# zkHubHQ/distributed-groth16

Hardware: AMD Instinct MI355X
Metric: groth16_constraints_per_sec (higher is better)
Workload: dtype u32; 1 GPU; BN254 Groth16 prove from the matrices, synthetic R1CS with 2^20 - 2 constraints (3 nonzeros per row of A and B), 2^20 wires, 2 instance variables; r, s != 0 (R1CS x witness + 6 NTTs of 2^20 + 4 G1 MSMs + 1 G2 MSM); proving key RESIDENT as window tables (built once per key outside the timed region); curve=bn254, log_domain=20, parallelism=single GPU, key_table_bytes=6039807360, key_table_stride=1

## Files before the change

### distributed-groth16_amd/csrc/ntt.hip

```cpp
#include <cstdio>
#include <cstdlib>
#include "ctx.h"
#include "fp29.h"
#include "types.h"

namespace dg16 {

static void optional_table_skipped(const char* what, size_t bytes) {
  static const bool verbose = [] { const char* e = getenv("DG16_VERBOSE"); return e && atoi(e) != 0; }();
  if (verbose) fprintf(stderr, "[dg16] %s (%zu bytes) not built: hipMalloc failed; using the composed form\n", what, bytes);
}


constexpr unsigned kTileLog = 10;
constexpr unsigned kTile = 1u << kTileLog;
constexpr unsigned kMaxStepLog = 10;
constexpr unsigned kLoBits = 11;

template <class F>
struct StepArgs {
  const F* src[3];
  F* dst[3];
  unsigned log_n, s, log_a, log_b;
  unsigned last;
  unsigned log_n1, log_n2;
  const F* small;
  unsigned sm;
  const F* tw_lo;
  const F* tw_hi;
  unsigned lb;
  const F* tw_full;
  const F* post_full;
  const F* pre_lo;
  const F* pre_hi;
  const F* post_lo;
  const F* post_hi;
  unsigned plb;
  const F* scale;
  unsigned src_piece_log, dst_piece_log;
  size_t src_piece_stride, dst_piece_stride;
};

__device__ __forceinline__ unsigned bitrev(unsigned v, unsigned bits) {
  return bits ? (__brev(v) >> (32 - bits)) : 0;
}

constexpr int kNttBound = 48 * 64;
constexpr int kNttIn = 128;
constexpr int kNttFirstOut = 9 * 64;
constexpr int kNttStepGrowth = 6 * 64 + 32;
constexpr int kNttOddGrowth = 3 * 64 + 32;
static_assert(kNttFirstOut + (int)((kMaxStepLog - 2) / 2) * kNttStepGrowth + kNttOddGrowth <= kNttBound,
              "NTT tile bound: a pass of kMaxStepLog levels can exceed kNttBound");

template <class F>
__global__ void __launch_bounds__(256) ntt_step_kernel(StepArgs<F> p) {
  using P = typename F::Params;
  using T = RR<P>;
  constexpr int N = T::N;
  using El = Fe<P, kNttBound, 1>;
  using Tw = Fe<P, 64, 1>;
  __shared__ uint32_t tile_w[kTile * N];
  constexpr int NLW = T::NL;
  __shared__ uint32_t tw_w[(1u << (kMaxStepLog - 1)) * NLW];
  static_assert((1u << (kMaxStepLog - 2)) * N <= (1u << (kMaxStepLog - 1)) * NLW, "unpacked twiddles of the shorter steps fit");
  const unsigned tid = threadIdx.x;
  const unsigned s = p.s;
  const unsigned nj = 1u << s;
  const unsigned log_t = (p.log_n < kTileLog ? p.log_n : kTileLog) - s;
  const unsigned Tn = 1u << log_t;
  const unsigned elems = nj << log_t;
  const size_t tile_id = blockIdx.x;
  auto slot = [](unsigned e) { return (e ^ ((e >> 2) & 31u)) * (unsigned)N; };
  auto ld_tile = [&](unsigned i) {
    El v;
    const unsigned o = slot(i);
#pragma unroll
    for (int j = 0; j < N; j++) v.l[j] = tile_w[o + j];
    return v;
  };
  auto st_tile = [&](unsigned i, const El& v) {
    const unsigned o = slot(i);
#pragma unroll
    for (int j = 0; j < N; j++) tile_w[o + j] = v.l[j];
  };
  const bool tw_packed = p.s == kMaxStepLog;
  auto ld_tw = [&](unsigned i) {
    if (tw_packed) return fe_from_words<P>(&tw_w[i * NLW]);
    Tw v;
#pragma unroll
    for (int j = 0; j < N; j++) v.l[j] = tw_w[i * N + j];
    return v;
  };
  auto ld_packed = [&](const F* ptr) { return fe_from_words<P>(ptr->l); };

  size_t a = 0, b0 = 0, k1_0 = 0, k2 = 0;
  if (!p.last) {
    const unsigned tiles_per_a_log = p.log_b - log_t;
    a = tile_id >> tiles_per_a_log;
    b0 = (tile_id & (((size_t)1 << tiles_per_a_log) - 1)) << log_t;
  } else {
    const unsigned k1_tiles_log = p.log_n1 - log_t;
    k2 = tile_id >> k1_tiles_log;
    k1_0 = (tile_id & (((size_t)1 << k1_tiles_log) - 1)) << log_t;
  }

  if (s >= 1)
    for (unsigned t = tid; t < (nj >> 1); t += 256) {
      const F* w = p.small + ((size_t)t << (p.sm - s));
      if (tw_packed) {
#pragma unroll
        for (int j = 0; j < NLW; j++) tw_w[t * NLW + j] = w->l[j];
      } else {
        const Tw u = ld_packed(w);
#pragma unroll
        for (int j = 0; j < N; j++) tw_w[t * N + j] = u.l[j];
      }
    }

  for (unsigned idx = tid; idx < elems; idx += 256) {
    unsigned n, t;
    size_t g;
    if (!p.last) {
      t = idx & (Tn - 1);
      n = idx >> log_t;
      g = ((((a << s) + n) << p.log_b) + b0 + t);
    } else {
      n = idx & (nj - 1);
      t = idx >> s;
      g = ((((k1_0 + t) << p.log_n2) + k2) << s) + n;
    }
    const size_t gs = p.src_piece_stride ? (g >> p.src_piece_log) * p.src_piece_stride + (g & (((size_t)1 << p.src_piece_log) - 1)) : g;
    const Tw x = ld_packed(p.src[blockIdx.y] + gs);
    El v = x.template as<kNttBound, 1>();
    if (p.pre_lo) {
      const auto w = ld_packed(p.pre_lo + (g & ((1u << p.plb) - 1))) * ld_packed(p.pre_hi + (g >> p.plb));
      v = (x * w).template as<kNttBound, 1>();
    }
    st_tile((bitrev(n, s) << log_t) + t, v);
  }
  __syncthreads();

  unsigned lv = 1;
  if (s >= 2) {
    using In = Fe<P, kNttIn, 1>;
    const Tw w3 = ld_tw(1u << (s - 2));
    for (unsigned q = tid; q < (elems >> 2); q += 256) {
      const unsigned t = q & (Tn - 1), pi = q >> log_t;
      const unsigned ia = (pi << (2 + log_t)) + t;
      const In xa = ld_tile(ia).template unsafe_assume<kNttIn, 1>(), xb = ld_tile(ia + Tn).template unsafe_assume<kNttIn, 1>(),
               xc = ld_tile(ia + 2 * Tn).template unsafe_assume<kNttIn, 1>(), xd = ld_tile(ia + 3 * Tn).template unsafe_assume<kNttIn, 1>();
      const auto a1 = xa + xb;
      const auto b1 = xa - xb;
      const auto c1 = xc + xd;
      const auto te = (xc - xd) * w3;
      const auto o0 = a1 + c1;
      const auto o2 = a1 - c1;
      const auto o1 = b1 + te;
      const auto o3 = b1 - te;
      static_assert(decltype(o0)::Bound <= kNttFirstOut && decltype(o1)::Bound <= kNttFirstOut &&
                    decltype(o2)::Bound <= kNttFirstOut && decltype(o3)::Bound <= kNttFirstOut, "first radix-4 step bound");
      st_tile(ia, norm(o0).template as<kNttBound, 1>());
      st_tile(ia + 2 * Tn, norm(o2).template as<kNttBound, 1>());
      st_tile(ia + Tn, norm(o1).template as<kNttBound, 1>());
      st_tile(ia + 3 * Tn, norm(o3).template as<kNttBound, 1>());
    }
    __syncthreads();
    lv = 3;
  }
  for (; lv + 1 <= s; lv += 2) {
    const unsigned half = 1u << (lv - 1);
    const unsigned sh1 = s - lv, sh2 = s - lv - 1;
    for (unsigned q = tid; q < (elems >> 2); q += 256) {
      const unsigned t = q & (Tn - 1), pi = q >> log_t;
      const unsigned k = pi & (half - 1), blk = pi >> (lv - 1);
      const unsigned ia = ((((blk << (lv + 1)) + k)) << log_t) + t;
      const unsigned st = half << log_t;
      const El xa = ld_tile(ia), xb = ld_tile(ia + st), xc = ld_tile(ia + 2 * st), xd = ld_tile(ia + 3 * st);
      const Tw w1 = ld_tw(k << sh1);
      const auto tb = xb * w1;
      const auto td = xd * w1;
      const auto a1 = xa + tb;
      const auto b1 = xa - tb;
      const auto c1 = xc + td;
      const auto d1 = xc - td;
      const auto tc = c1 * ld_tw(k << sh2);
      const auto te = d1 * ld_tw((k + half) << sh2);
      const auto o0 = a1 + tc;
      const auto o2 = a1 - tc;
      const auto o1 = b1 + te;
      const auto o3 = b1 - te;
      static_assert(decltype(o0)::Bound - kNttBound <= kNttStepGrowth && decltype(o1)::Bound - kNttBound <= kNttStepGrowth &&
                    decltype(o2)::Bound - kNttBound <= kNttStepGrowth && decltype(o3)::Bound - kNttBound <= kNttStepGrowth,
                    "radix-4 step growth");
      st_tile(ia, norm(o0).template unsafe_assume<kNttBound, 1>());
      st_tile(ia + 2 * st, norm(o2).template unsafe_assume<kNttBound, 1>());
      st_tile(ia + st, norm(o1).template unsafe_assume<kNttBound, 1>());
      st_tile(ia + 3 * st, norm(o3).template unsafe_assume<kNttBound, 1>());
    }
    __syncthreads();
  }
  if (lv == s) {
    const unsigned half = 1u << (s - 1);
    for (unsigned q = tid; q < (elems >> 1); q += 256) {
      const unsigned t = q & (Tn - 1), k = q >> log_t;
      const unsigned i0 = (k << log_t) + t, i1 = i0 + (half << log_t);
      const El x = ld_tile(i0);
      const auto ty = ld_tile(i1) * ld_tw(k);
      const auto o0 = x + ty;
      const auto o1 = x - ty;
      static_assert(decltype(o0)::Bound - kNttBound <= kNttOddGrowth && decltype(o1)::Bound - kNttBound <= kNttOddGrowth,
                    "odd level growth");
      st_tile(i0, norm(o0).template unsafe_assume<kNttBound, 1>());
      st_tile(i1, norm(o1).template unsafe_assume<kNttBound, 1>());
    }
    __syncthreads();
  }

  for (unsigned idx = tid; idx < elems; idx += 256) {
    unsigned t = idx & (Tn - 1);
    unsigned k = idx >> log_t;
    const El v = ld_tile((k << log_t) + t);
    Fe<P, 64, 1> out;
    size_t g;
    if (!p.last) {
      size_t b = b0 + t;
      size_t e = (b * k) << p.log_a;
      if (p.tw_full) {
        if (e || p.scale) out = canon(v * ld_packed(p.tw_full + (((size_t)k << p.log_b) + b)));
        else out = canon(v);
      } else if (e) {
        const auto w = ld_packed(p.tw_lo + (e & ((1u << p.lb) - 1))) * ld_packed(p.tw_hi + (e >> p.lb));
        out = canon(v * w);
      } else if (p.scale) {
        out = canon(v * ld_packed(p.tw_hi));
      } else {
        out = canon(v);
      }
      g = ((((a << s) + k) << p.log_b) + b);
    } else {
      g = (k1_0 + t) + (k2 << p.log_n1) + ((size_t)k << (p.log_n1 + p.log_n2));
      if (p.post_full) {
        const auto w = ld_packed(p.post_full + g);
        if (p.scale) out = canon((v * ld_packed(p.scale)) * w);
        else out = canon(v * w);
      } else if (p.scale && p.post_lo) {
        const auto w = ld_packed(p.post_lo + (g & ((1u << p.plb) - 1))) * ld_packed(p.post_hi + (g >> p.plb));
        out = canon((v * ld_packed(p.scale)) * w);
      } else if (p.scale) {
        out = canon(v * ld_packed(p.scale));
      } else if (p.post_lo) {
        const auto w = ld_packed(p.post_lo + (g & ((1u << p.plb) - 1))) * ld_packed(p.post_hi + (g >> p.plb));
        out = canon(v * w);
      } else {
        out = canon(v);
      }
    }
    F o;
    fe_to_words<P>(out, o.l);
    if (p.dst_piece_stride) g = (g >> p.dst_piece_log) * p.dst_piece_stride + (g & (((size_t)1 << p.dst_piece_log) - 1));
    p.dst[blockIdx.y][g] = o;
  }
}

template <class F>
__global__ void to_internal_kernel(F* t, size_t count) {
  size_t j = (size_t)blockIdx.x * blockDim.x + threadIdx.x;
  if (j >= count) return;
  using P = typename F::Params;
  F c;
#pragma unroll
  for (int i = 0; i < F::NL; i++) c.l[i] = RR<P>::R_WORDS.v[i];
  t[j] = t[j] * c;
}
template <class F>
static void* internal_copy(hipStream_t s, const void* src, size_t count) {
  void* d = nullptr;
  DG_HIP(hipMalloc(&d, count * sizeof(F)));
  DG_HIP(hipMemcpyAsync(d, src, count * sizeof(F), hipMemcpyDeviceToDevice, s));
  hipLaunchKernelGGL(to_internal_kernel<F>, dim3((unsigned)((count + 255) / 256)), dim3(256), 0, s, (F*)d, count);
  return d;
}

template <class F>
__global__ void powers_kernel(F* out, size_t count, unsigned shift, const F* base_ptr,
                              unsigned root_log, int invert, const F* c_ptr) {
  size_t j = (size_t)blockIdx.x * blockDim.x + threadIdx.x;
  if (j >= count) return;
  F base;
  if (base_ptr) {
    base = *base_ptr;
  } else {
    F w;
#pragma unroll
    for (int i = 0; i < F::NL; i++) w.l[i] = F::Params::TWO_ADIC_ROOT[i];
    for (unsigned i = root_log; i < (unsigned)F::Params::TWO_ADICITY; i++) w = w.sqr();
    if (invert) {
      F acc = F::one(), sq = w;
      for (unsigned i = 0; i < root_log; i++) { acc = acc * sq; sq = sq.sqr(); }
      w = acc;
    }
    base = w;
  }
  F r = base.pow_u64((uint64_t)j << shift);
  if (c_ptr) r = r * *c_ptr;
  out[j] = r;
}

template <class F>
__global__ void n_inv_kernel(F* out, unsigned log_n) {
  F two = F::one() + F::one();
  F half = two.inv();
  *out = half.pow_u64(log_n);
}

struct Plan {
  unsigned nsteps;
  unsigned s[3];
};
static Plan make_plan(unsigned log_n) {
  Plan pl{};
  if (log_n <= kTileLog && log_n <= kMaxStepLog) {
    pl.nsteps = 1;
    pl.s[0] = log_n;
  } else if (log_n <= 2 * kMaxStepLog) {
    pl.nsteps = 2;
    pl.s[0] = log_n / 2;
    pl.s[1] = log_n - pl.s[0];
  } else {
    pl.nsteps = 3;
    pl.s[0] = log_n / 3;
    pl.s[1] = (log_n - pl.s[0]) / 2;
    pl.s[2] = log_n - pl.s[0] - pl.s[1];
  }
  return pl;
}

constexpr unsigned kFullTwiddleMaxLog = 24;
inline unsigned full_twiddle_min_log() {
  static const unsigned v = [] { const char* e = getenv("DG16_NTT_TABLE_MIN_LOG"); return e ? (unsigned)atoi(e) : 21u; }();
  return v;
}
template <class F>
__global__ void __launch_bounds__(256) full_twiddle_kernel(F* __restrict__ out, size_t count, unsigned log_a, unsigned log_b,
                                                            const F* __restrict__ lo, const F* __restrict__ hi, unsigned lb) {
  using P = typename F::Params;
  const size_t idx = (size_t)blockIdx.x * blockDim.x + threadIdx.x;
  if (idx >= count) return;
  const size_t k = idx >> log_b, b = idx & (((size_t)1 << log_b) - 1);
  const size_t e = (b * k) << log_a;
  const auto w = fe_from_words<P>(lo[e & (((size_t)1 << lb) - 1)].l) * fe_from_words<P>(hi[e >> lb].l);
  F o;
  fe_to_words<P>(canon(w), o.l);
  out[idx] = o;
}
template <class F>
__global__ void __launch_bounds__(256) flat_powers_kernel(F* __restrict__ out, size_t count, const F* __restrict__ lo,
                                                           const F* __restrict__ hi, unsigned lb) {
  using P = typename F::Params;
  const size_t o = (size_t)blockIdx.x * blockDim.x + threadIdx.x;
  if (o >= count) return;
  const auto w = fe_from_words<P>(lo[o & (((size_t)1 << lb) - 1)].l) * fe_from_words<P>(hi[o >> lb].l);
  F r;
  fe_to_words<P>(canon(w), r.l);
  out[o] = r;
}

template <class F>
static const TwiddleSet& get_twiddles(Call& k, int curve, unsigned log_n, int inverse) {
  std::lock_guard<std::mutex> g(k.ctx->mu);
  TwiddleKey key{curve, log_n, inverse};
  auto it = k.ctx->twiddles.find(key);
  if (it != k.ctx->twiddles.end()) return it->second;
  TwiddleSet ts;
  ts.lb = log_n < kLoBits ? log_n : kLoBits;
  ts.sm = log_n < kMaxStepLog ? (log_n ? log_n : 1) : kMaxStepLog;
  size_t nlo = (size_t)1 << ts.lb, nhi = (size_t)1 << (log_n - ts.lb), nsm = (size_t)1 << (ts.sm - 1);
  DG_HIP(hipMalloc(&ts.lo, nlo * sizeof(F)));
  DG_HIP(hipMalloc(&ts.hi, nhi * sizeof(F)));
  DG_HIP(hipMalloc(&ts.small, nsm * sizeof(F)));
  DG_HIP(hipMalloc(&ts.n_inv, sizeof(F)));
  hipStream_t s = k.s();
  hipLaunchKernelGGL(n_inv_kernel<F>, dim3(1), dim3(1), 0, s, (F*)ts.n_inv, log_n);
  hipLaunchKernelGGL(powers_kernel<F>, dim3((unsigned)((nlo + 255) / 256)), dim3(256), 0, s, (F*)ts.lo,
                     nlo, 0u, (const F*)nullptr, log_n, inverse, (const F*)nullptr);
  hipLaunchKernelGGL(powers_kernel<F>, dim3((unsigned)((nhi + 255) / 256)), dim3(256), 0, s, (F*)ts.hi,
                     nhi, ts.lb, (const F*)nullptr, log_n, inverse, (const F*)nullptr);
  if (inverse) {
    DG_HIP(hipMalloc(&ts.hi_scaled, nhi * sizeof(F)));
    hipLaunchKernelGGL(powers_kernel<F>, dim3((unsigned)((nhi + 255) / 256)), dim3(256), 0, s,
                       (F*)ts.hi_scaled, nhi, ts.lb, (const F*)nullptr, log_n, inverse,
                       (const F*)ts.n_inv);
  }
  hipLaunchKernelGGL(powers_kernel<F>, dim3((unsigned)((nsm + 255) / 256)), dim3(256), 0, s, (F*)ts.small,
                     nsm, log_n >= ts.sm ? log_n - ts.sm : 0, (const F*)nullptr, log_n ? log_n : 1, inverse,
                     (const F*)nullptr);
  ts.lo_i = internal_copy<F>(s, ts.lo, nlo);
  ts.hi_i = internal_copy<F>(s, ts.hi, nhi);
  if (inverse) ts.hi_scaled_i = internal_copy<F>(s, ts.hi_scaled, nhi);
  ts.small_i = internal_copy<F>(s, ts.small, nsm);
  ts.n_inv_i = internal_copy<F>(s, ts.n_inv, 1);
  {
    const Plan pl = make_plan(log_n);
    unsigned consumed = 0;
    for (unsigned j = 0; j + 1 < pl.nsteps && log_n <= kFullTwiddleMaxLog && log_n >= full_twiddle_min_log(); j++) {
      const size_t cnt = (size_t)1 << (log_n - consumed);
      if (hipMalloc(&ts.full[j], cnt * sizeof(F)) != hipSuccess) {
        (void)hipGetLastError();
        ts.full[j] = nullptr;
        optional_table_skipped("inter-step twiddle table", cnt * sizeof(F));
        consumed += pl.s[j];
        continue;
      }
      hipLaunchKernelGGL(full_twiddle_kernel<F>, dim3((unsigned)((cnt + 255) / 256)), dim3(256), 0, s, (F*)ts.full[j], cnt,
                         consumed, log_n - consumed - pl.s[j], (const F*)ts.lo_i,
                         (const F*)((inverse && j == 0) ? ts.hi_scaled_i : ts.hi_i), ts.lb);
      consumed += pl.s[j];
    }
  }
  DG_HIP(hipGetLastError());
  DG_HIP(hipStreamSynchronize(s));
  return k.ctx->twiddles.emplace(key, ts).first->second;
}

template <class F>
static void build_power_tables(Call& k, const F* g_dev, unsigned log_n, F* lo, F* hi, unsigned lb) {
  size_t nlo = (size_t)1 << lb, nhi = (size_t)1 << (log_n - lb);
  hipLaunchKernelGGL(powers_kernel<F>, dim3((unsigned)((nlo + 255) / 256)), dim3(256), 0, k.s(), lo, nlo, 0u,
                     g_dev, 0u, 0, (const F*)nullptr);
  hipLaunchKernelGGL(powers_kernel<F>, dim3((unsigned)((nhi + 255) / 256)), dim3(256), 0, k.s(), hi, nhi, lb,
                     g_dev, 0u, 0, (const F*)nullptr);
  hipLaunchKernelGGL(to_internal_kernel<F>, dim3((unsigned)((nlo + 255) / 256)), dim3(256), 0, k.s(), lo, nlo);
  hipLaunchKernelGGL(to_internal_kernel<F>, dim3((unsigned)((nhi + 255) / 256)), dim3(256), 0, k.s(), hi, nhi);
  DG_HIP(hipGetLastError());
}

template <class F>
__global__ void inv_one_kernel(F* out, const F* in) { *out = in->inv(); }

template <class F>
static void ntt_run_batch(Call& k, int curve, unsigned nb, const F* const* in, F* const* data, F* const* tmp,
                          unsigned log_n, int inverse, const F* pre_lo, const F* pre_hi, const F* post_lo,
                          const F* post_hi, unsigned plb, unsigned src_piece_log = 0, size_t src_piece_stride = 0,
                          unsigned dst_piece_log = 0, size_t dst_piece_stride = 0, const F* post_full = nullptr) {
  DG_REQUIRE(log_n <= 3 * kMaxStepLog, DG16_ERR_UNSUPPORTED, "log_n > 27 not supported yet");
  DG_REQUIRE(nb >= 1 && nb <= 3, DG16_ERR_BAD_ARG, "1..3 transforms per batch");
  const TwiddleSet& ts = get_twiddles<F>(k, curve, log_n, inverse);
  Plan pl = make_plan(log_n);
  unsigned consumed = 0;
  for (unsigned j = 0; j < pl.nsteps; j++) {
    StepArgs<F> a{};
    a.log_n = log_n;
    a.s = pl.s[j];
    a.log_a = consumed;
    a.log_b = log_n - consumed - pl.s[j];
    a.last = (j == pl.nsteps - 1);
    a.log_n1 = pl.nsteps >= 2 ? pl.s[0] : 0;
    a.log_n2 = pl.nsteps == 3 ? pl.s[1] : 0;
    a.small = (const F*)ts.small_i;
    a.sm = ts.sm;
    a.tw_lo = (const F*)ts.lo_i;
    bool fold_scale = inverse && pl.nsteps > 1 && j == 0;
    a.tw_hi = (const F*)(fold_scale ? ts.hi_scaled_i : ts.hi_i);
    a.lb = ts.lb;
    a.tw_full = (!a.last && j < 2) ? (const F*)ts.full[j] : nullptr;
    a.scale = nullptr;
    if (fold_scale) a.scale = (const F*)ts.n_inv_i;
    if (inverse && pl.nsteps == 1) a.scale = (const F*)ts.n_inv_i;
    if (j == 0) { a.pre_lo = pre_lo; a.pre_hi = pre_hi; a.src_piece_log = src_piece_log; a.src_piece_stride = src_piece_stride; }
    if (a.last) { a.post_lo = post_lo; a.post_hi = post_hi; a.post_full = post_full; a.dst_piece_log = dst_piece_log; a.dst_piece_stride = dst_piece_stride; }
    a.plb = plb;
    for (unsigned i = 0; i < nb; i++) {
      a.src[i] = j == 0 ? in[i] : tmp[i];
      a.dst[i] = (pl.nsteps == 1 || a.last) ? data[i] : tmp[i];
    }
    unsigned log_tile = log_n < kTileLog ? log_n : kTileLog;
    size_t blocks = (size_t)1 << (log_n - log_tile);
    if (a.last && pl.nsteps > 1) {
      unsigned log_t = log_tile - a.s;
      DG_REQUIRE(a.log_n1 >= log_t, DG16_ERR_UNSUPPORTED, "plan violates N1 >= T");
    } else if (!a.last) {
      unsigned log_t = log_tile - a.s;
      DG_REQUIRE(a.log_b >= log_t, DG16_ERR_UNSUPPORTED, "plan violates B >= T");
    }
    hipLaunchKernelGGL(ntt_step_kernel<F>, dim3((unsigned)blocks, nb), dim3(256), 0, k.s(), a);
    DG_HIP(hipGetLastError());
    consumed += pl.s[j];
  }
}
template <class F>
static void ntt_run(Call& k, int curve, F* data, F* tmp, unsigned log_n, int inverse,
                    const F* pre_lo, const F* pre_hi, const F* post_lo, const F* post_hi, unsigned plb) {
  const F* in[1] = {data};
  F* d[1] = {data};
  F* t[1] = {tmp};
  ntt_run_batch<F>(k, curve, 1, in, d, t, log_n, inverse, pre_lo, pre_hi, post_lo, post_hi, plb);
}

template <class F>
static void ntt_typed(Call& k, int curve, void* data, unsigned log_n, int inverse, const void* coset_host) {
  F* d = (F*)data;
  F* tmp = (F*)ws(k.c, 8, sizeof(F) << log_n);
  const F *pre_lo = nullptr, *pre_hi = nullptr, *post_lo = nullptr, *post_hi = nullptr;
  unsigned plb = log_n < kLoBits ? log_n : kLoBits;
  if (coset_host) {
    F* g = (F*)ws(k.c, 9, 2 * sizeof(F));
    DG_HIP(hipMemcpyAsync(g, coset_host, sizeof(F), hipMemcpyHostToDevice, k.s()));
    F* lo = (F*)ws(k.c, 10, sizeof(F) << plb);
    F* hi = (F*)ws(k.c, 11, sizeof(F) << (log_n - plb));
    if (inverse) {
      hipLaunchKernelGGL(inv_one_kernel<F>, dim3(1), dim3(1), 0, k.s(), g + 1, g);
      build_power_tables<F>(k, g + 1, log_n, lo, hi, plb);
      post_lo = lo; post_hi = hi;
    } else {
      build_power_tables<F>(k, g, log_n, lo, hi, plb);
      pre_lo = lo; pre_hi = hi;
    }
  }
  k.begin_dominant();
  ntt_run<F>(k, curve, d, tmp, log_n, inverse, pre_lo, pre_hi, post_lo, post_hi, plb);
  k.end_dominant();
}

const TwiddleSet& get_twiddles_any(Call& k, int curve, unsigned log_n, int inverse) {
  switch (curve) {
    case 0: return get_twiddles<bn254_fr>(k, curve, log_n, inverse);
    case 1: return get_twiddles<bls12_381_fr>(k, curve, log_n, inverse);
    default: return get_twiddles<bls12_377_fr>(k, curve, log_n, inverse);
  }
}

void ntt_launch(Call& k, int curve, void* data, unsigned log_n, int inverse, const void* coset_host) {
  switch (curve) {
    case 0: ntt_typed<bn254_fr>(k, curve, data, log_n, inverse, coset_host); break;
    case 1: ntt_typed<bls12_381_fr>(k, curve, data, log_n, inverse, coset_host); break;
    default: ntt_typed<bls12_377_fr>(k, curve, data, log_n, inverse, coset_host); break;
  }
}

template <class F>
__global__ void __launch_bounds__(256) mul_sub_kernel(const F* __restrict__ a, const F* __restrict__ b,
                                                       const F* __restrict__ c, F* __restrict__ out, size_t n) {
  size_t stride = (size_t)gridDim.x * blockDim.x;
  for (size_t i = (size_t)blockIdx.x * blockDim.x + threadIdx.x; i < n; i += stride)
    out[i] = a[i] * b[i] - c[i];
}

template <class F>
static const F* flat_shift_table(Call& k, const TwiddleSet& t2, unsigned log_m) {
  std::lock_guard<std::mutex> g(k.ctx->mu);
  TwiddleSet& w = const_cast<TwiddleSet&>(t2);
  if (!w.shift_full && !w.shift_full_tried) {
    w.shift_full_tried = true;
    const size_t m = (size_t)1 << log_m;
    if (hipMalloc(&w.shift_full, m * sizeof(F)) != hipSuccess) {
      (void)hipGetLastError();
      w.shift_full = nullptr;
      optional_table_skipped("w_2m shift table", m * sizeof(F));
      return nullptr;
    }
    hipLaunchKernelGGL(flat_powers_kernel<F>, dim3((unsigned)((m + 255) / 256)), dim3(256), 0, k.s(), (F*)w.shift_full, m,
                       (const F*)t2.lo_i, (const F*)t2.hi_i, t2.lb);
    DG_HIP(hipGetLastError());
    DG_HIP(hipStreamSynchronize(k.s()));
  }
  return (const F*)w.shift_full;
}

template <class F>
static void h_poly_typed(Call& k, int curve, const void* a, const void* b, const void* c, unsigned log_m,
                         void* out) {
  size_t bytes = sizeof(F) << log_m;
  F* v[3] = {(F*)ws(k.c, 12, bytes), (F*)ws(k.c, 13, bytes), (F*)ws(k.c, 14, bytes)};
  F* t0 = (F*)ws(k.c, 8, 3 * bytes);
  F* tmp[3] = {t0, t0 + ((size_t)1 << log_m), t0 + ((size_t)2 << log_m)};
  const F* in[3] = {(const F*)a, (const F*)b, (const F*)c};
  const TwiddleSet& t2 = get_twiddles<F>(k, curve, log_m + 1, 0);
  const F* shift = log_m <= kFullTwiddleMaxLog && log_m >= full_twiddle_min_log() ? flat_shift_table<F>(k, t2, log_m) : nullptr;
  k.begin_dominant();
  ntt_run_batch<F>(k, curve, 3, in, v, tmp, log_m, 1, nullptr, nullptr, (const F*)t2.lo_i, (const F*)t2.hi_i, t2.lb,
                   0, 0, 0, 0, shift);
  ntt_run_batch<F>(k, curve, 3, v, v, tmp, log_m, 0, nullptr, nullptr, nullptr, nullptr, 0);
  size_t n = (size_t)1 << log_m;
  size_t blocks = (n + 255) / 256;
  size_t cap = (size_t)k.ctx->compute_units * 8;
  if (blocks > cap) blocks = cap;
  hipLaunchKernelGGL(mul_sub_kernel<F>, dim3((unsigned)blocks), dim3(256), 0, k.s(), v[0], v[1], v[2], (F*)out, n);
  DG_HIP(hipGetLastError());
  k.end_dominant();
}


template <class F>
__device__ __forceinline__ F tw_lookup(const F* lo, const F* hi, unsigned lb, size_t e) {
  const size_t l = e & (((size_t)1 << lb) - 1), h = e >> lb;
  if (l == 0) return hi[h];
  if (h == 0) return lo[l];
  return lo[l] * hi[h];
}

template <int LOGN, class F>
__device__ __forceinline__ void small_dft(F* x, const F* roots) {
  constexpr int N = 1 << LOGN;
#pragma unroll
  for (int i = 0; i < N; i++) {
    int j = 0;
#pragma unroll
    for (int b = 0; b < LOGN; b++) j |= ((i >> b) & 1) << (LOGN - 1 - b);
    if (j > i) { const F t = x[i]; x[i] = x[j]; x[j] = t; }
  }
#pragma unroll
  for (int lv = 1; lv <= LOGN; lv++) {
    constexpr int dummy = 0; (void)dummy;
    const int half = 1 << (lv - 1);
#pragma unroll
    for (int q = 0; q < N / 2; q++) {
      const int kk = q & (half - 1), blk = q >> (lv - 1);
      const int i0 = (blk << lv) + kk, i1 = i0 + half;
      const F y = kk ? x[i1] * roots[kk << (LOGN - lv)] : x[i1];
      const F u = x[i0];
      x[i0] = u + y;
      x[i1] = u - y;
    }
  }
}

struct CrossArgs {
  const void *wi_lo, *wi_hi, *wf_lo, *wf_hi, *g_lo, *g_hi, *n_inv;
  unsigned wlb, glb;
  unsigned log_m, rank;
  size_t S;
};

template <class F, int LOGN>
__global__ void __launch_bounds__(256) hdist_cross_kernel(const F* __restrict__ in, F* __restrict__ out, CrossArgs p) {
  constexpr int N = 1 << LOGN;
  const size_t j = (size_t)blockIdx.x * blockDim.x + threadIdx.x;
  if (j >= p.S) return;
  const unsigned v = blockIdx.y;
  const size_t M = p.S << LOGN;
  const size_t k2 = (size_t)p.rank * p.S + j;
  const F *wi_lo = (const F*)p.wi_lo, *wi_hi = (const F*)p.wi_hi, *wf_lo = (const F*)p.wf_lo, *wf_hi = (const F*)p.wf_hi;
  const F *g_lo = (const F*)p.g_lo, *g_hi = (const F*)p.g_hi;
  F x[N];
#pragma unroll
  for (int i = 0; i < N; i++) x[i] = in[((size_t)i * 3 + v) * p.S + j];
  {
    const F base = tw_lookup(wi_lo, wi_hi, p.wlb, k2);
    F pw = base;
#pragma unroll
    for (int i = 1; i < N; i++) {
      x[i] = x[i] * pw;
      if (i + 1 < N) pw = pw * base;
    }
  }
  F roots[N / 2 ? N / 2 : 1];
#pragma unroll
  for (int t = 0; t < N / 2; t++) roots[t] = tw_lookup(wi_lo, wi_hi, p.wlb, M * t);
  small_dft<LOGN>(x, roots);
  {
    const F gm = tw_lookup(g_lo, g_hi, p.glb, M);
    F pw = tw_lookup(g_lo, g_hi, p.glb, k2) * *(const F*)p.n_inv;
#pragma unroll
    for (int i = 0; i < N; i++) {
      x[i] = x[i] * pw;
      if (i + 1 < N) pw = pw * gm;
    }
  }
#pragma unroll
  for (int t = 0; t < N / 2; t++) roots[t] = tw_lookup(wf_lo, wf_hi, p.wlb, M * t);
  small_dft<LOGN>(x, roots);
  {
    const F base = tw_lookup(wf_lo, wf_hi, p.wlb, k2);
    F pw = base;
#pragma unroll
    for (int i = 1; i < N; i++) {
      x[i] = x[i] * pw;
      if (i + 1 < N) pw = pw * base;
    }
  }
#pragma unroll
  for (int i = 0; i < N; i++) out[((size_t)i * 3 + v) * p.S + j] = x[i];
}

template <class F, int LOGN>
__global__ void __launch_bounds__(256) ntt_dist_cross_kernel(const F* __restrict__ in, F* __restrict__ out, const F* w_lo,
                                                              const F* w_hi, unsigned wlb, const F* n_inv, unsigned rank,
                                                              size_t S) {
  constexpr int N = 1 << LOGN;
  const size_t j = (size_t)blockIdx.x * blockDim.x + threadIdx.x;
  if (j >= S) return;
  const size_t M = S << LOGN, k2 = (size_t)rank * S + j;
  F x[N];
#pragma unroll
  for (int i = 0; i < N; i++) x[i] = in[(size_t)i * S + j];
  {
    const F base = tw_lookup(w_lo, w_hi, wlb, k2);
    F pw = base;
#pragma unroll
    for (int i = 1; i < N; i++) {
      x[i] = x[i] * pw;
      if (i + 1 < N) pw = pw * base;
    }
  }
  F roots[N / 2 ? N / 2 : 1];
#pragma unroll
  for (int t = 0; t < N / 2; t++) roots[t] = tw_lookup(w_lo, w_hi, wlb, M * t);
  small_dft<LOGN>(x, roots);
#pragma unroll
  for (int i = 0; i < N; i++) out[(size_t)i * S + j] = n_inv ? x[i] * *n_inv : x[i];
}

static unsigned log2_exact(unsigned n) {
  unsigned l = 0;
  while ((1u << l) < n) l++;
  DG_REQUIRE((1u << l) == n, DG16_ERR_BAD_ARG, "rank count must be a power of two");
  return l;
}

template <class F>
static void h_poly_dist_stage_typed(Call& k, int curve, unsigned log_m, unsigned rank, unsigned n_ranks, int stage,
                                    const void* const* in, void* out) {
  const unsigned log_n = log2_exact(n_ranks);
  DG_REQUIRE(log_n >= 1 && log_n <= 3, DG16_ERR_UNSUPPORTED, "sharded h-polynomial: 2, 4 or 8 ranks");
  DG_REQUIRE(log_m >= 2 * log_n, DG16_ERR_BAD_ARG, "sharded h-polynomial: domain smaller than ranks^2");
  DG_REQUIRE(rank < n_ranks, DG16_ERR_BAD_ARG, "rank out of range");
  const unsigned log_M = log_m - log_n, log_S = log_M - log_n;
  const size_t M = (size_t)1 << log_M, S = (size_t)1 << log_S;
  F* t0 = (F*)ws(k.c, 8, 3 * M * sizeof(F));
  F* tmp[3] = {t0, t0 + M, t0 + 2 * M};
  if (stage == 0) {
    const F* src[3] = {(const F*)in[0], (const F*)in[1], (const F*)in[2]};
    F* dst[3] = {(F*)out, (F*)out + S, (F*)out + 2 * S};
    ntt_run_batch<F>(k, curve, 3, src, dst, tmp, log_M, 1, nullptr, nullptr, nullptr, nullptr, 0, 0, 0, log_S, 3 * S);
  } else if (stage == 1) {
    const TwiddleSet& wi = get_twiddles<F>(k, curve, log_m, 1);
    const TwiddleSet& wf = get_twiddles<F>(k, curve, log_m, 0);
    const TwiddleSet& g = get_twiddles<F>(k, curve, log_m + 1, 0);
    const TwiddleSet& nn = get_twiddles<F>(k, curve, log_n, 1);
    CrossArgs a{wi.lo, wi.hi, wf.lo, wf.hi, g.lo, g.hi, nn.n_inv, wi.lb, g.lb, log_m, rank, S};
    dim3 grid((unsigned)((S + 255) / 256), 3);
    switch (log_n) {
      case 1: hipLaunchKernelGGL((hdist_cross_kernel<F, 1>), grid, dim3(256), 0, k.s(), (const F*)in[0], (F*)out, a); break;
      case 2: hipLaunchKernelGGL((hdist_cross_kernel<F, 2>), grid, dim3(256), 0, k.s(), (const F*)in[0], (F*)out, a); break;
      default: hipLaunchKernelGGL((hdist_cross_kernel<F, 3>), grid, dim3(256), 0, k.s(), (const F*)in[0], (F*)out, a); break;
    }
    DG_HIP(hipGetLastError());
  } else {
    const F* base = (const F*)in[0];
    const F* src[3] = {base, base + S, base + 2 * S};
    F* v0 = (F*)ws(k.c, 12, 3 * M * sizeof(F));
    F* v[3] = {v0, v0 + M, v0 + 2 * M};
    ntt_run_batch<F>(k, curve, 3, src, v, tmp, log_M, 0, nullptr, nullptr, nullptr, nullptr, 0, log_S, 3 * S, 0, 0);
    size_t blocks = (M + 255) / 256;
    size_t cap = (size_t)k.ctx->compute_units * 8;
    if (blocks > cap) blocks = cap;
    hipLaunchKernelGGL(mul_sub_kernel<F>, dim3((unsigned)blocks), dim3(256), 0, k.s(), v[0], v[1], v[2], (F*)out, M);
    DG_HIP(hipGetLastError());
  }
}

template <class F>
static void ntt_dist_stage_typed(Call& k, int curve, unsigned log_n_total, unsigned rank, unsigned n_ranks, int inverse,
                                 int stage, const void* in, void* out) {
  const unsigned log_n = log2_exact(n_ranks);
  DG_REQUIRE(log_n >= 1 && log_n <= 3, DG16_ERR_UNSUPPORTED, "sharded NTT: 2, 4 or 8 ranks");
  DG_REQUIRE(log_n_total >= 2 * log_n, DG16_ERR_BAD_ARG, "sharded NTT: domain smaller than ranks^2");
  DG_REQUIRE(rank < n_ranks, DG16_ERR_BAD_ARG, "rank out of range");
  const unsigned log_M = log_n_total - log_n;
  const size_t M = (size_t)1 << log_M, S = M >> log_n;
  if (stage == 0) {
    F* tmp = (F*)ws(k.c, 8, M * sizeof(F));
    const F* src[1] = {(const F*)in};
    F* dst[1] = {(F*)out};
    F* t[1] = {tmp};
    ntt_run_batch<F>(k, curve, 1, src, dst, t, log_M, inverse, nullptr, nullptr, nullptr, nullptr, 0);
  } else {
    const TwiddleSet& w = get_twiddles<F>(k, curve, log_n_total, inverse);
    const F* n_inv = inverse ? (const F*)get_twiddles<F>(k, curve, log_n, 1).n_inv : nullptr;
    dim3 grid((unsigned)((S + 255) / 256));
#define DG_NDX(L)                                                                                                   \
  hipLaunchKernelGGL((ntt_dist_cross_kernel<F, L>), grid, dim3(256), 0, k.s(), (const F*)in, (F*)out, (const F*)w.lo, \
                     (const F*)w.hi, w.lb, n_inv, rank, S)
    switch (log_n) {
      case 1: DG_NDX(1); break;
      case 2: DG_NDX(2); break;
      default: DG_NDX(3); break;
    }
#undef DG_NDX
    DG_HIP(hipGetLastError());
  }
}
void ntt_dist_stage(Call& k, int curve, unsigned log_n_total, unsigned rank, unsigned n_ranks, int inverse, int stage,
                    const void* in, void* out) {
  switch (curve) {
    case 0: ntt_dist_stage_typed<bn254_fr>(k, curve, log_n_total, rank, n_ranks, inverse, stage, in, out); break;
    case 1: ntt_dist_stage_typed<bls12_381_fr>(k, curve, log_n_total, rank, n_ranks, inverse, stage, in, out); break;
    default: ntt_dist_stage_typed<bls12_377_fr>(k, curve, log_n_total, rank, n_ranks, inverse, stage, in, out); break;
  }
}
void ntt_dist_launch(Call& k, int curve, const dg16_comm* comm, const void* in, void* out, unsigned log_n_total,
                     int inverse) {
  const unsigned n = comm->n_ranks(comm->self), rank = comm->rank(comm->self);
  const size_t bytes = (((size_t)1 << log_n_total) / n) * 32;
  void* buf_a = ws(k.c, 26, bytes);
  void* buf_b = ws(k.c, 27, bytes);
  ntt_dist_stage(k, curve, log_n_total, rank, n, inverse, 0, in, buf_a);
  int rc = comm->all_to_all(comm->self, buf_a, buf_b, bytes / n, k.s());
  DG_REQUIRE(rc == DG16_OK, DG16_ERR_NET, "all-to-all of the sharded NTT failed");
  ntt_dist_stage(k, curve, log_n_total, rank, n, inverse, 1, buf_b, out);
}

void h_poly_dist_stage(Call& k, int curve, unsigned log_m, unsigned rank, unsigned n_ranks, int stage,
                       const void* const* in, void* out) {
  switch (curve) {
    case 0: h_poly_dist_stage_typed<bn254_fr>(k, curve, log_m, rank, n_ranks, stage, in, out); break;
    case 1: h_poly_dist_stage_typed<bls12_381_fr>(k, curve, log_m, rank, n_ranks, stage, in, out); break;
    default: h_poly_dist_stage_typed<bls12_377_fr>(k, curve, log_m, rank, n_ranks, stage, in, out); break;
  }
}

void h_poly_dist_launch(Call& k, int curve, const dg16_comm* comm, const void* a, const void* b, const void* c,
                        unsigned log_m, void* out) {
  const unsigned n = comm->n_ranks(comm->self), rank = comm->rank(comm->self);
  const size_t M = ((size_t)1 << log_m) / n, bytes = 3 * M * 32;
  void* buf_a = ws(k.c, 26, bytes);
  void* buf_b = ws(k.c, 27, bytes);
  const void* rows[3] = {a, b, c};
  h_poly_dist_stage(k, curve, log_m, rank, n, 0, rows, buf_a);
  int rc = comm->all_to_all(comm->self, buf_a, buf_b, bytes / n, k.s());
  DG_REQUIRE(rc == DG16_OK, DG16_ERR_NET, "all-to-all of the sharded h-polynomial failed");
  const void* in1[1] = {buf_b};
  h_poly_dist_stage(k, curve, log_m, rank, n, 1, in1, buf_a);
  rc = comm->all_to_all(comm->self, buf_a, buf_b, bytes / n, k.s());
  DG_REQUIRE(rc == DG16_OK, DG16_ERR_NET, "all-to-all of the sharded h-polynomial failed");
  h_poly_dist_stage(k, curve, log_m, rank, n, 2, in1, out);
}

void h_poly_launch(Call& k, int curve, const void* a, const void* b, const void* c, unsigned log_m, void* out) {
  switch (curve) {
    case 0: h_poly_typed<bn254_fr>(k, curve, a, b, c, log_m, out); break;
    case 1: h_poly_typed<bls12_381_fr>(k, curve, a, b, c, log_m, out); break;
    default: h_poly_typed<bls12_377_fr>(k, curve, a, b, c, log_m, out); break;
  }
}

}
```

Before: 105.9 million constraints/s.

## Add radix-8/16 register-blocked NTT step kernel with lazy reduction

Adds a new NTT step kernel that performs several butterfly levels (up to 3 or 4) per pass in registers before writing back to a swizzled shared-memory tile. This cuts the number of shared-memory round trips and barriers per step, and uses bound tracking to skip modular normalisation between levels. The kernel runs with 128 lanes and a waves-per-EU hint, and is enabled by default for sizes of at least 2^10, with an environment variable to turn it off. The gain is limited to the NTT part of the prove, and the new code carries more register pressure and more complex bound logic.

```diff
diff --git a/distributed-groth16_amd/csrc/ntt.hip b/distributed-groth16_amd/csrc/ntt.hip
--- a/distributed-groth16_amd/csrc/ntt.hip
+++ b/distributed-groth16_amd/csrc/ntt.hip
@@ -1,5 +1,6 @@
 #include <cstdio>
 #include <cstdlib>
+#include <type_traits>
 #include "ctx.h"
 #include "fp29.h"
 #include "types.h"
@@ -263,6 +264,251 @@
   }
 }
 
+constexpr int kNttFirstLevels = 3;
+constexpr int kNttMaxLevels = 4;
+constexpr int kNttTripFirstOut = 23 * 64;
+constexpr int kNttLevelGrowth = 3 * 64 + 32;
+static_assert(kNttTripFirstOut + (int)(kMaxStepLog - kNttFirstLevels) * kNttLevelGrowth <= kNttBound,
+              "NTT tile bound: a pass of kMaxStepLog levels can exceed kNttBound");
+
+constexpr unsigned kNttLanes = 128;
+
+__host__ __device__ constexpr unsigned ntt_trip_levels(unsigned r, bool first) {
+  if (first) return r < (unsigned)kNttFirstLevels ? r : (unsigned)kNttFirstLevels;
+  return r == (unsigned)kNttMaxLevels ? r : (r < 3 ? r : 3);
+}
+
+template <class A, class B>
+struct NttTypeMax {
+  static constexpr int Bound = A::Bound > B::Bound ? A::Bound : B::Bound;
+  static constexpr int Limb = A::Limb > B::Limb ? A::Limb : B::Limb;
+};
+template <class X, bool First>
+struct NttPlainPair {
+  static constexpr int Bound = 0, Limb = 0;
+};
+template <class X>
+struct NttPlainPair<X, true> : NttTypeMax<decltype(X() + X()), decltype(X() - X())> {};
+template <class P, int B, int L, bool First>
+struct NttLevel {
+  using X = Fe<P, B, L>;
+  using Prod = decltype(X() * Fe<P, 64, 1>());
+  using WithProduct = NttTypeMax<decltype(X() + Prod()), decltype(X() - Prod())>;
+  using Plain = NttPlainPair<X, First>;
+  static constexpr int OB = Plain::Bound > WithProduct::Bound ? Plain::Bound : WithProduct::Bound;
+  static constexpr int OL = Plain::Limb > WithProduct::Limb ? Plain::Limb : WithProduct::Limb;
+  using Out = Fe<P, OB, OL>;
+};
+template <class P, int L, bool First>
+constexpr bool ntt_level_needs_norm() {
+  return L > 1 && ((First ? 2 * L + 2 : L + 3) > RR<P>::LIMBCAP || !rr_cols_fit<P>(L));
+}
+
+template <class P, int K, bool First>
+struct NttTrip {
+  static constexpr int R = 1 << K;
+  template <int LV, class X, class TwF, class Sink>
+  static __device__ __forceinline__ void run(const X (&x)[R], TwF&& tw, Sink&& sink) {
+    if constexpr (LV == K) {
+      if constexpr (First) static_assert(X::Bound <= kNttTripFirstOut - (kNttFirstLevels - K) * kNttLevelGrowth, "first trip bound");
+#pragma unroll
+      for (int j = 0; j < R; j++) sink(j, x[j]);
+    } else if constexpr (ntt_level_needs_norm<P, X::Limb, First>()) {
+      Fe<P, X::Bound, 1> y[R];
+#pragma unroll
+      for (int j = 0; j < R; j++) y[j] = norm(x[j]);
+      run<LV>(y, tw, sink);
+    } else {
+      using Lv = NttLevel<P, X::Bound, X::Limb, First>;
+      static_assert(First || Lv::OB - X::Bound <= kNttLevelGrowth, "level growth");
+      typename Lv::Out y[R];
+      constexpr int h = 1 << LV;
+#pragma unroll
+      for (int jl = 0; jl < h; jl++) {
+        if (First && jl == 0) {
+          if constexpr (First) {
+#pragma unroll
+            for (int j = 0; j < R; j += 2 * h) {
+              y[j] = (x[j] + x[j + h]).template as<Lv::OB, Lv::OL>();
+              y[j + h] = (x[j] - x[j + h]).template as<Lv::OB, Lv::OL>();
+            }
+          }
+        } else {
+          const Fe<P, 64, 1> w = tw(LV, jl);
+#pragma unroll
+          for (int j = jl; j < R; j += 2 * h) {
+            const auto t = x[j + h] * w;
+            y[j] = (x[j] + t).template as<Lv::OB, Lv::OL>();
+            y[j + h] = (x[j] - t).template as<Lv::OB, Lv::OL>();
+          }
+        }
+      }
+      run<LV + 1>(y, tw, sink);
+    }
+  }
+};
+
+template <class F>
+__global__ void __launch_bounds__(kNttLanes) __attribute__((amdgpu_waves_per_eu(2))) ntt_trip_kernel(StepArgs<F> p) {
+  using P = typename F::Params;
+  using T = RR<P>;
+  constexpr int N = T::N;
+  using El = Fe<P, kNttBound, 1>;
+  using Tw = Fe<P, 64, 1>;
+  __shared__ uint32_t tile_w[kTile * N];
+  const unsigned tid = threadIdx.x;
+  const unsigned s = p.s;
+  const unsigned nj = 1u << s;
+  const unsigned log_t = (p.log_n < kTileLog ? p.log_n : kTileLog) - s;
+  const unsigned Tn = 1u << log_t;
+  const unsigned elems = nj << log_t;
+  const size_t tile_id = blockIdx.x;
+  auto slot = [](unsigned e) { return (e ^ (((e >> 3) ^ (e >> 5)) & 31u)) * (unsigned)N; };
+  auto ld_tile = [&](unsigned i) {
+    El v;
+    const unsigned o = slot(i);
+#pragma unroll
+    for (int j = 0; j < N; j++) v.l[j] = tile_w[o + j];
+    return v;
+  };
+  auto st_tile = [&](unsigned i, const El& v) {
+    const unsigned o = slot(i);
+#pragma unroll
+    for (int j = 0; j < N; j++) tile_w[o + j] = v.l[j];
+  };
+  auto ld_packed = [&](const F* ptr) { return fe_from_words<P>(ptr->l); };
+
+  size_t a = 0, b0 = 0, k1_0 = 0, k2 = 0;
+  if (!p.last) {
+    const unsigned tiles_per_a_log = p.log_b - log_t;
+    a = tile_id >> tiles_per_a_log;
+    b0 = (tile_id & (((size_t)1 << tiles_per_a_log) - 1)) << log_t;
+  } else {
+    const unsigned k1_tiles_log = p.log_n1 - log_t;
+    k2 = tile_id >> k1_tiles_log;
+    k1_0 = (tile_id & (((size_t)1 << k1_tiles_log) - 1)) << log_t;
+  }
+
+  for (unsigned idx = tid; idx < elems; idx += kNttLanes) {
+    unsigned n, t;
+    size_t g;
+    if (!p.last) {
+      t = idx & (Tn - 1);
+      n = idx >> log_t;
+      g = ((((a << s) + n) << p.log_b) + b0 + t);
+    } else {
+      n = idx & (nj - 1);
+      t = idx >> s;
+      g = ((((k1_0 + t) << p.log_n2) + k2) << s) + n;
+    }
+    const size_t gs = p.src_piece_stride ? (g >> p.src_piece_log) * p.src_piece_stride + (g & (((size_t)1 << p.src_piece_log) - 1)) : g;
+    const Tw x = ld_packed(p.src[blockIdx.y] + gs);
+    El v = x.template as<kNttBound, 1>();
+    if (p.pre_lo) {
+      const auto w = ld_packed(p.pre_lo + (g & ((1u << p.plb) - 1))) * ld_packed(p.pre_hi + (g >> p.plb));
+      const auto xw = x * w;
+      static_assert(decltype(xw)::Bound <= kNttIn, "a load times a table entry is a fresh value");
+      v = xw.template as<kNttBound, 1>();
+    }
+    st_tile((bitrev(n, s) << log_t) + t, v);
+  }
+  __syncthreads();
+
+  auto trip = [&](auto kc, auto fc, unsigned lv) {
+    constexpr int K = decltype(kc)::value;
+    constexpr bool First = decltype(fc)::value;
+    constexpr int R = 1 << K;
+    using In = Fe<P, First ? kNttIn : kNttBound, 1>;
+    const unsigned half = 1u << (lv - 1);
+    const unsigned st = half << log_t;
+    for (unsigned q = tid; q < (elems >> K); q += kNttLanes) {
+      const unsigned t = q & (Tn - 1), pi = q >> log_t;
+      const unsigned k = pi & (half - 1), blk = pi >> (lv - 1);
+      const unsigned ia = (((blk << (lv - 1 + K)) + k) << log_t) + t;
+      In x[R];
+#pragma unroll
+      for (int j = 0; j < R; j++) x[j] = ld_tile(ia + j * st).template unsafe_assume<First ? kNttIn : kNttBound, 1>();
+      NttTrip<P, K, First>::template run<0>(
+          x,
+          [&](int l, int jl) {
+            const F* w = p.small + ((size_t)((k + jl * half) << (s - lv - l)) << (p.sm - s));
+            return ld_packed(w);
+          },
+          [&](int j, const auto& o) {
+            if constexpr (First) st_tile(ia + j * st, norm(o).template as<kNttBound, 1>());
+            else st_tile(ia + j * st, norm(o).template unsafe_assume<kNttBound, 1>());
+          });
+    }
+    __syncthreads();
+  };
+  {
+    using std::integral_constant;
+    using std::false_type;
+    using std::true_type;
+    unsigned lv = 1;
+    if (s >= 1) {
+      switch (ntt_trip_levels(s, true)) {
+        case 1: trip(integral_constant<int, 1>(), true_type(), lv); lv += 1; break;
+        case 2: trip(integral_constant<int, 2>(), true_type(), lv); lv += 2; break;
+        default: trip(integral_constant<int, 3>(), true_type(), lv); lv += 3; break;
+      }
+    }
+    while (lv <= s) {
+      switch (ntt_trip_levels(s - lv + 1, false)) {
+        case 1: trip(integral_constant<int, 1>(), false_type(), lv); lv += 1; break;
+        case 2: trip(integral_constant<int, 2>(), false_type(), lv); lv += 2; break;
+        case 3: trip(integral_constant<int, 3>(), false_type(), lv); lv += 3; break;
+        default: trip(integral_constant<int, 4>(), false_type(), lv); lv += 4; break;
+      }
+    }
+  }
+
+  for (unsigned idx = tid; idx < elems; idx += kNttLanes) {
+    unsigned t = idx & (Tn - 1);
+    unsigned k = idx >> log_t;
+    const El v = ld_tile((k << log_t) + t);
+    Fe<P, 64, 1> out;
+    size_t g;
+    if (!p.last) {
+      size_t b = b0 + t;
+      size_t e = (b * k) << p.log_a;
+      if (p.tw_full) {
+        if (e || p.scale) out = canon(v * ld_packed(p.tw_full + (((size_t)k << p.log_b) + b)));
+        else out = canon(v);
+      } else if (e) {
+        const auto w = ld_packed(p.tw_lo + (e & ((1u << p.lb) - 1))) * ld_packed(p.tw_hi + (e >> p.lb));
+        out = canon(v * w);
+      } else if (p.scale) {
+        out = canon(v * ld_packed(p.tw_hi));
+      } else {
+        out = canon(v);
+      }
+      g = ((((a << s) + k) << p.log_b) + b);
+    } else {
+      g = (k1_0 + t) + (k2 << p.log_n1) + ((size_t)k << (p.log_n1 + p.log_n2));
+      if (p.post_full) {
+        const auto w = ld_packed(p.post_full + g);
+        if (p.scale) out = canon((v * ld_packed(p.scale)) * w);
+        else out = canon(v * w);
+      } else if (p.scale && p.post_lo) {
+        const auto w = ld_packed(p.post_lo + (g & ((1u << p.plb) - 1))) * ld_packed(p.post_hi + (g >> p.plb));
+        out = canon((v * ld_packed(p.scale)) * w);
+      } else if (p.scale) {
+        out = canon(v * ld_packed(p.scale));
+      } else if (p.post_lo) {
+        const auto w = ld_packed(p.post_lo + (g & ((1u << p.plb) - 1))) * ld_packed(p.post_hi + (g >> p.plb));
+        out = canon(v * w);
+      } else {
+        out = canon(v);
+      }
+    }
+    F o;
+    fe_to_words<P>(out, o.l);
+    if (p.dst_piece_stride) g = (g >> p.dst_piece_log) * p.dst_piece_stride + (g & (((size_t)1 << p.dst_piece_log) - 1));
+    p.dst[blockIdx.y][g] = o;
+  }
+}
+
 template <class F>
 __global__ void to_internal_kernel(F* t, size_t count) {
   size_t j = (size_t)blockIdx.x * blockDim.x + threadIdx.x;
@@ -366,6 +612,10 @@
   out[o] = r;
 }
 
+inline bool ntt_use_trips() {
+  static const bool v = [] { const char* e = getenv("DG16_NTT_TRIPS"); return !e || atoi(e) != 0; }();
+  return v;
+}
 template <class F>
 static const TwiddleSet& get_twiddles(Call& k, int curve, unsigned log_n, int inverse) {
   std::lock_guard<std::mutex> g(k.ctx->mu);
@@ -483,7 +733,10 @@
       unsigned log_t = log_tile - a.s;
       DG_REQUIRE(a.log_b >= log_t, DG16_ERR_UNSUPPORTED, "plan violates B >= T");
     }
-    hipLaunchKernelGGL(ntt_step_kernel<F>, dim3((unsigned)blocks, nb), dim3(256), 0, k.s(), a);
+    if (log_n >= kTileLog && ntt_use_trips())
+      hipLaunchKernelGGL(ntt_trip_kernel<F>, dim3((unsigned)blocks, nb), dim3(kNttLanes), 0, k.s(), a);
+    else
+      hipLaunchKernelGGL(ntt_step_kernel<F>, dim3((unsigned)blocks, nb), dim3(256), 0, k.s(), a);
     DG_HIP(hipGetLastError());
     consumed += pl.s[j];
   }
```

Result: slower. 102.3 million constraints/s (-3.4%).
